# kristi700/ViT-SSL

Measured on AMD Instinct MI355X. Metric: images_per_sec, higher is better.
Workload: dtype bf16; 1 GPU; ViT-B/16 SimMIM 224x224 mask 0.6 dropout 0.1 AdamW, batch 256/GPU; global_batch=256, parallelism=dp1

## Files before the change

vit-ssl_amd/csrc/attention.hip:

```cpp
#include <stdlib.h>
#include "common.h"
#include "attention_tiles.h"
#include "attention_bwd.h"

#ifdef VITSSL_ATTN_STAMPS
__device__ unsigned long long* g_attn_stamps = nullptr;
#define ATTN_STAMP(i)                                                                                   \
  do {                                                                                                  \
    if (g_attn_stamps && threadIdx.x == 0) g_attn_stamps[(size_t)blockIdx.x * 4 + (i)] = __builtin_amdgcn_s_memrealtime(); \
  } while (0)
#else
#define ATTN_STAMP(i) \
  do {                \
  } while (0)
#endif

namespace {

using namespace vitssl_attn;

__device__ __forceinline__ void startup_stagger(int first_round_wgs, int window_ticks) {
  if (window_ticks <= 0 || (int)blockIdx.x >= first_round_wgs) return;
  if (threadIdx.x < 64) {
    const unsigned h = (blockIdx.x * 2654435761u) >> 20;
    const unsigned long long delay = (unsigned long long)window_ticks * h >> 12;
    const unsigned long long t0 = __builtin_amdgcn_s_memrealtime();
    while (__builtin_amdgcn_s_memrealtime() - t0 < delay) __builtin_amdgcn_s_sleep(8);
  }
  __syncthreads();
}


__device__ __forceinline__ f32x4 key_mask_init(int kt, int g, int N) {
  f32x4 v;
#pragma unroll
  for (int r = 0; r < 4; ++r) v[r] = (kt * 16 + 4 * g + r < N) ? 0.f : -INFINITY;
  return v;
}

template <int NKT>
__device__ __forceinline__ void softmax_tile(f32x4 (&s)[NKT], float& m_out, float& sum_out) {
  float m = -INFINITY;
#pragma unroll
  for (int kt = 0; kt < NKT; ++kt) m = fmaxf(fmaxf(m, fmaxf(s[kt][0], s[kt][1])), fmaxf(s[kt][2], s[kt][3]));
  m = fmaxf(m, __shfl_xor(m, 16, 64));
  m = fmaxf(m, __shfl_xor(m, 32, 64));
  const float mc = -m * SCALE_LOG2E;
  const f32x4 c4 = {SCALE_LOG2E, SCALE_LOG2E, SCALE_LOG2E, SCALE_LOG2E}, m4 = {mc, mc, mc, mc};
  f32x4 part = {0.f, 0.f, 0.f, 0.f};
#pragma unroll
  for (int kt = 0; kt < NKT; ++kt) {
    const f32x4 e = __builtin_elementwise_fma(s[kt], c4, m4);
#pragma unroll
    for (int r = 0; r < 4; ++r) s[kt][r] = __builtin_amdgcn_exp2f(e[r]);
    part += s[kt];
  }
  float sum = (part[0] + part[1]) + (part[2] + part[3]);
  sum += __shfl_xor(sum, 16, 64);
  sum += __shfl_xor(sum, 32, 64);
  m_out = m;
  sum_out = sum;
}

template <int NS, int NW>
__global__ __launch_bounds__(64 * NW, 2) void attn_fwd_kernel(const bf16_t* __restrict__ qkv, bf16_t* __restrict__ out,
                                                          float* __restrict__ lse, float* __restrict__ probs, int N, int H,
                                                          int stagger_wgs, int stagger_ticks, unsigned char* __restrict__ out8) {
  extern __shared__ __attribute__((aligned(16))) char smem[];
  constexpr int Np = 32 * NS;
  constexpr int NKT = 2 * NS;
  startup_stagger(stagger_wgs, stagger_ticks);
  char* Kt = smem;
  char* Vt = smem + Np * ROWB;
  const int b = blockIdx.x / H, h = blockIdx.x - b * H;
  const long long stride = 3LL * H * DH;
  const bf16_t* qg = qkv + (long long)b * N * stride + h * DH;
  const bf16_t* kg = qg + (long long)H * DH;
  const bf16_t* vg = kg + (long long)H * DH;
  const int lane = threadIdx.x & 63;
  const int wave = __builtin_amdgcn_readfirstlane(threadIdx.x >> 6);
  const int g = lane >> 4, li = lane & 15;
  const int nqp = (N + 31) >> 5;
  const f32x4 zero4 = {0.f, 0.f, 0.f, 0.f};
  const f32x4 tail0 = key_mask_init(NKT - 2, g, N), tail1 = key_mask_init(NKT - 1, g, N);

  ATTN_STAMP(0);
  bf16x8 qn[2][2];
#pragma unroll
  for (int t = 0; t < 2; ++t) {
    qn[t][0] = glb_frag(qg, stride, wave * 32 + t * 16 + li, 0, N, lane);
    qn[t][1] = glb_frag(qg, stride, wave * 32 + t * 16 + li, 1, N, lane);
  }
  dma_tile<NW>(Kt, kg, stride, N, Np, wave, lane);
  asm volatile("s_waitcnt vmcnt(0)" ::: "memory");
  __builtin_amdgcn_s_barrier();
  dma_tile<NW>(Vt, vg, stride, N, Np, wave, lane);
  ATTN_STAMP(1);

  const int iters = (nqp + NW - 1) / NW;
  for (int it = 0; it < iters; ++it) {
    const int qp = wave + NW * it;
    const bool active = qp < nqp;
    const int q[2] = {qp * 32 + li, qp * 32 + 16 + li};
    bf16x8 qf[2][2];
#pragma unroll
    for (int t = 0; t < 2; ++t) {
      qf[t][0] = qn[t][0];
      qf[t][1] = qn[t][1];
    }
    if (it + 1 < iters) {
#pragma unroll
      for (int t = 0; t < 2; ++t) {
// ... 123 lines not shown
#pragma unroll
    for (int t = 0; t < QT; ++t)
#pragma unroll
      for (int kk = 0; kk < 2; ++kk)
        qq[t][kk] = __builtin_bit_cast(bf16x8, __builtin_amdgcn_raw_buffer_load_b128(
                                                   rq, (unsigned)((long long)q[t] * stride * 2 + 64 * kk + 16 * g), 0, 0));
  };
  constexpr unsigned OOB = 0x80000000u;
  const unsigned out_bytes = (unsigned)((long long)N * H * DH * 2);
  unsigned vrel[4];
  {
    const int tq = (lane >> 2) & 3, tpp = lane & 3;
#pragma unroll
    for (int dt = 0; dt < 4; ++dt) vrel[dt] = (unsigned)(tile_off(4 * g + tq, 2 * dt + (tpp >> 1)) + 8 * (tpp & 1));
  }

  bf16x8 qn[QT][2];
  issue_tiles(item, smem, smem + TILE);
  load_q(item, qn);
  bool first = true;
#ifdef VITSSL_ATTN_STAMPS
  unsigned long long seg[6] = {0, 0, 0, 0, 0, 0};
  unsigned long long tprev = __builtin_amdgcn_s_memrealtime();
#define PSTAMP(i)                                                   \
  do {                                                              \
    __builtin_amdgcn_sched_barrier(0);                              \
    const unsigned long long tn_ = __builtin_amdgcn_s_memrealtime(); \
    seg[i] += tn_ - tprev;                                          \
    tprev = tn_;                                                    \
    __builtin_amdgcn_sched_barrier(0);                              \
  } while (0)
#else
#define PSTAMP(i) \
  do {            \
  } while (0)
#endif

  auto one_item = [&](auto cur_c) {
    constexpr int cur = decltype(cur_c)::value;
    const char* Kt = smem + cur * 2 * TILE;
    const char* Vt = Kt + TILE;
    char* Kn = smem + (cur ^ 1) * 2 * TILE;
    const int b = item / H, h = item - b * H;
    const int next = item + (int)gridDim.x;
    const bool has_next = next < nitems;
    if (probs || first || !active) __builtin_amdgcn_s_waitcnt(0x0F70);
    else if (out8) __builtin_amdgcn_s_waitcnt(0x0F70 | (QT * 7));
    else __builtin_amdgcn_s_waitcnt(0x0F70 | (QT * 3));
    first = false;
    __builtin_amdgcn_s_barrier();
    PSTAMP(0);
    bf16x8 qf[QT][2];
#pragma unroll
    for (int t = 0; t < QT; ++t) {
      qf[t][0] = qn[t][0];
      qf[t][1] = qn[t][1];
    }
    if (has_next) {
      issue_tiles(next, Kn, Kn + TILE);
      load_q(next, qn);
    }
    if (active) {
      f32x4 sc[QT][NKT];
#pragma unroll
      for (int kt = 0; kt < NKT; ++kt) {
        const bf16x8 k0 = lds_frag(Kt, kt * 16 + li, 0, lane);
        const bf16x8 k1 = lds_frag(Kt, kt * 16 + li, 1, lane);
#pragma unroll
        for (int t = 0; t < QT; ++t) sc[t][kt] = MFMA16(k0, qf[t][0], kt == NKT - 2 ? tail0 : (kt == NKT - 1 ? tail1 : zero4));
#pragma unroll
        for (int t = 0; t < QT; ++t) sc[t][kt] = MFMA16(k1, qf[t][1], sc[t][kt]);
      }
      PSTAMP(1);
      float m[QT], sum[QT], inv[QT];
#pragma unroll
      for (int t = 0; t < QT; ++t) softmax_tile<NKT>(sc[t], m[t], sum[t]);
      PSTAMP(2);
      __amdgpu_buffer_rsrc_t rl = __builtin_amdgcn_make_buffer_rsrc((void*)(lse + ((long long)b * H + h) * N), 0, N * 4, 0x00020000);
#pragma unroll
      for (int t = 0; t < QT; ++t) {
        inv[t] = 1.0f / sum[t];
        __builtin_amdgcn_raw_buffer_store_b32(__float_as_uint(m[t] * SCALE + __logf(sum[t])), rl, g == 0 ? (unsigned)q[t] * 4u : OOB, 0, 0);
        if (probs && q[t] < N) {
          int qrow = q[t];
          asm volatile("" : "+v"(qrow));
          float* pr = probs + (((long long)b * H + h) * N + qrow) * N;
#pragma unroll
          for (int kt = 0; kt < NKT; ++kt)
#pragma unroll
            for (int r = 0; r < 4; ++r) {
              const int key = kt * 16 + 4 * g + r;
              if (key < N) pr[key] = sc[t][kt][r] * inv[t];
            }
        }
      }
      f32x4 o[QT][4];
#pragma unroll
      for (int t = 0; t < QT; ++t)
#pragma unroll
        for (int dt = 0; dt < 4; ++dt) o[t][dt] = f32x4{0.f, 0.f, 0.f, 0.f};
      const unsigned vbase = (unsigned)(size_t)LDS_PTR(Vt);
      unsigned va[4];
#pragma unroll
      for (int dt = 0; dt < 4; ++dt) va[dt] = vbase + vrel[dt];
      constexpr int SETS = QT == 2 ? 2 : 1;
      s16x4 lo[SETS][4], hi[SETS][4];
      if constexpr (SETS == 2) tr_read_v4<0>(lo[0], hi[0], va);
      static_for<NS>([&](auto st_c) {
        constexpr int st = decltype(st_c)::value;
        constexpr int set = SETS == 2 ? (st & 1) : 0;
        bf16x8 pf[QT];
#pragma unroll
        for (int t = 0; t < QT; ++t) pf[t] = pack_frag(sc[t][2 * st], sc[t][2 * st + 1]);
        if constexpr (SETS == 1) {
          tr_read_v4<st>(lo[0], hi[0], va);
          asm volatile("s_waitcnt lgkmcnt(0)" ::: "memory");
        } else if constexpr (st + 1 < NS) {
          tr_read_v4<st + 1>(lo[set ^ 1], hi[set ^ 1], va);
          asm volatile("s_waitcnt lgkmcnt(8)" ::: "memory");
        } else {
          asm volatile("s_waitcnt lgkmcnt(0)" ::: "memory");
        }
        __builtin_amdgcn_sched_barrier(0);
#pragma unroll
        for (int dt = 0; dt < 4; ++dt) {
          typedef __attribute__((ext_vector_type(8))) short s16x8;
          const s16x8 v = {lo[set][dt][0], lo[set][dt][1], lo[set][dt][2], lo[set][dt][3], hi[set][dt][0], hi[set][dt][1], hi[set][dt][2], hi[set][dt][3]};
          const bf16x8 vf = __builtin_bit_cast(bf16x8, v);
#pragma unroll
          for (int t = 0; t < QT; ++t) o[t][dt] = MFMA16(vf, pf[t], o[t][dt]);
        }
      });
      PSTAMP(3);
      __amdgpu_buffer_rsrc_t ro = __builtin_amdgcn_make_buffer_rsrc((void*)(out + (long long)b * N * (H * DH)), 0, (int)out_bytes, 0x00020000);
      char* xw = smem + 4 * TILE + wave * 2048;
      const int rho = lane >> 3, kap = lane & 7;
      const unsigned tw = (unsigned)(li * 128 + ((g ^ (2 * (li >> 1))) << 3));
      const unsigned tr = (unsigned)(rho * 128 + ((kap ^ (rho >> 1)) << 4));
#pragma unroll
      for (int t = 0; t < QT; ++t) {
#pragma unroll
        for (int dt = 0; dt < 4; ++dt) *(u32x2*)(xw + (tw ^ (unsigned)(32 * dt))) = pack4(o[t][dt] * inv[t]);
        const u32x4 s1 = *(const u32x4*)(xw + tr), s2 = *(const u32x4*)(xw + ((tr + 1024u) ^ 64u));
        const unsigned rowoff = (unsigned)((wave * QT + t) * 16 + rho) * (unsigned)(H * DH * 2) + (unsigned)(h * DH * 2 + 16 * kap);
        __builtin_amdgcn_raw_buffer_store_b128(s1, ro, rowoff, 0, 0);
        __builtin_amdgcn_raw_buffer_store_b128(s2, ro, rowoff + 8u * (unsigned)(H * DH * 2), 0, 0);
      }
      if (out8) {
        __amdgpu_buffer_rsrc_t r8 = __builtin_amdgcn_make_buffer_rsrc((void*)(out8 + (long long)b * N * (H * DH)), 0, (int)(out_bytes / 2), 0x00020000);
#pragma unroll
        for (int t = 0; t < QT; ++t)
#pragma unroll
          for (int dt = 0; dt < 4; ++dt) {
            const f32x4 v = o[t][dt] * inv[t];
            __builtin_amdgcn_raw_buffer_store_b32(pack_fp8x4(v[0], v[1], v[2], v[3]), r8,
                                                  (unsigned)q[t] * (unsigned)(H * DH) + (unsigned)(h * DH + 4 * g + 16 * dt), 0, 0);
          }
      }
    }
    PSTAMP(4);
#ifdef VITSSL_ATTN_STAMPS
    seg[5] += 1;
#endif
    item = next;
    return has_next;
  };
  for (;;) {
    if (!one_item(IC<0>{})) break;
    if (!one_item(IC<1>{})) break;
  }
#ifdef VITSSL_ATTN_STAMPS
  if (g_attn_stamps && threadIdx.x == 0)
    for (int i = 0; i < 6; ++i) g_attn_stamps[(size_t)blockIdx.x * 8 + i] = seg[i];
#endif
#undef PSTAMP
}

template <int NS, int NW>
__global__ __launch_bounds__(64 * NW, 2) void attn_bwd_fused_kernel(const bf16_t* __restrict__ qkv, const bf16_t* __restrict__ outp,
                                                             const bf16_t* __restrict__ dout, const float* __restrict__ lse,
                                                             bf16_t* __restrict__ dqkv, int N, int H, int stagger_wgs,
                                                             int stagger_ticks, unsigned char* __restrict__ dq8,
                                                             const float* __restrict__ qscale, float* qamax) {
  extern __shared__ __attribute__((aligned(16))) char smem[];
  constexpr int Np = 32 * NS;
  constexpr int SROW = SX_ROW<NS>;
  const float qsc = (dq8 && qscale) ? *qscale : 1.0f;
  float qmax = 0.f;
  startup_stagger(stagger_wgs, stagger_ticks);
  char* Qt = smem;
  char* Dt = Qt + Np * ROWB;
  char* Kt = Dt + Np * ROWB;
  char* Sx = Kt + Np * ROWB;
  float* lse_s = (float*)(Sx + 2 * 32 * SROW);
  float* del_s = lse_s + Np;
  const int b = blockIdx.x / H, h = blockIdx.x - b * H;
  const long long stride = 3LL * H * DH, ostride = (long long)H * DH;
  const bf16_t* qg = qkv + (long long)b * N * stride + h * DH;
  const bf16_t* kg = qg + (long long)H * DH;
  const bf16_t* vg = kg + (long long)H * DH;
  const bf16_t* dog = dout + (long long)b * N * ostride + h * DH;
  const bf16_t* og = outp + (long long)b * N * ostride + h * DH;
  const int lane = threadIdx.x & 63;
  const int wave = __builtin_amdgcn_readfirstlane(threadIdx.x >> 6);
  const int g = lane >> 4, li = lane & 15;
  const bool has_keys = wave < NS;

  ATTN_STAMP(0);
  char* Ot = Sx;
  dma_tile<NW>(Qt, qg, stride, N, Np, wave, lane);
  dma_tile<NW>(Dt, dog, ostride, N, Np, wave, lane);
  dma_tile<NW>(Kt, kg, stride, N, Np, wave, lane);
  dma_tile<NW>(Ot, og, ostride, N, Np, wave, lane);
  bf16x8 kf[2][2], vf[2][2];
  f32x4 kinit[2];
  if (has_keys) {
#pragma unroll
    for (int kt = 0; kt < 2; ++kt) {
      const int key = wave * 32 + kt * 16 + li;
      kinit[kt] = key_mask_init1(key, N);
#pragma unroll
      for (int kk = 0; kk < 2; ++kk) vf[kt][kk] = glb_frag(vg, stride, key, kk, N, lane);
    }
  }
  float lrow[(Np + 32 * NW - 1) / (32 * NW)];
#pragma unroll
  for (int it = 0; it < (Np + 32 * NW - 1) / (32 * NW); ++it) {
    const int row = (threadIdx.x >> 1) + it * 32 * NW;
    lrow[it] = row < N ? lse[((long long)b * H + h) * N + row] : 0.f;
  }
  asm volatile("s_waitcnt vmcnt(0)" ::: "memory");
  __syncthreads();
  if (has_keys) {
#pragma unroll
    for (int kt = 0; kt < 2; ++kt)
#pragma unroll
      for (int kk = 0; kk < 2; ++kk) kf[kt][kk] = lds_frag(Kt, wave * 32 + kt * 16 + li, kk, lane);
  }
#pragma unroll
// ... 349 lines not shown
      }
    }
  }
  dq_tile(Sx + ((NS - 1) & 1) * 32 * SROW, NS - 1);
  ATTN_STAMP(2);
  if (has_keys) {
#pragma unroll
    for (int kt = 0; kt < 2; ++kt) {
      const int key = wave * 32 + kt * 16 + li;
      if (dqkv) {
        char* xw = Qt + wave * 2048;
        const int rho = lane >> 3, kap = lane & 7;
        const unsigned tw = (unsigned)(li * 128 + ((g ^ (2 * (li >> 1))) << 3));
        const unsigned tr = (unsigned)(rho * 128 + ((kap ^ (rho >> 1)) << 4));
        const int key_a = wave * 32 + kt * 16 + rho;
        bf16_t* dka = dqkv + ((long long)b * N + key_a) * stride + (long long)H * DH + h * DH + 8 * kap;
#pragma unroll
        for (int tsel = 0; tsel < 2; ++tsel) {
#pragma unroll
          for (int dt = 0; dt < 4; ++dt) *(u32x2*)(xw + (tw ^ (unsigned)(32 * dt))) = pack4(tsel == 0 ? dk[dt][kt] : dv[dt][kt]);
          const u32x4 s1 = *(const u32x4*)(xw + tr), s2 = *(const u32x4*)(xw + ((tr + 1024u) ^ 64u));
          bf16_t* dst = dka + (long long)tsel * H * DH;
          if (key_a < N) *(u32x4*)dst = s1;
          if (key_a + 8 < N) *(u32x4*)(dst + 8 * stride) = s2;
        }
      }
      if (dq8) {
        unsigned qk[4], qv[4];
#pragma unroll
        for (int dt = 0; dt < 4; ++dt) {
          const f32x4 a = dk[dt][kt], c = dv[dt][kt];
          qk[dt] = pack_fp8x4(a[0] * qsc, a[1] * qsc, a[2] * qsc, a[3] * qsc);
          qv[dt] = pack_fp8x4(c[0] * qsc, c[1] * qsc, c[2] * qsc, c[3] * qsc);
          if (key < N) {
            qmax = fmaxf(qmax, fmaxf(fmaxf(fabsf(a[0]), fabsf(a[1])), fmaxf(fabsf(a[2]), fabsf(a[3]))));
            qmax = fmaxf(qmax, fmaxf(fmaxf(fabsf(c[0]), fabsf(c[1])), fmaxf(fabsf(c[2]), fabsf(c[3]))));
          }
        }
        const u32x4 rk = lane_rows_transpose4(qk), rv = lane_rows_transpose4(qv);
        if (key < N) {
          unsigned char* k8 = dq8 + ((long long)b * N + key) * stride + (long long)H * DH + h * DH + 16 * g;
          *(u32x4*)k8 = rk;
          *(u32x4*)(k8 + (long long)H * DH) = rv;
        }
      }
    }
  }
  if (dq8 && qamax) publish_amax(qmax, qamax, lane);
#ifdef VITSSL_ATTN_STAMPS
  asm volatile("s_waitcnt vmcnt(0)" ::: "memory");
#endif
  ATTN_STAMP(3);
}


template <int NS, bool Q8>
__global__ __launch_bounds__(512) void attn_bwd_pers_kernel(const bf16_t* __restrict__ qkv, const bf16_t* __restrict__ outp,
                                                            const bf16_t* __restrict__ dout, const float* __restrict__ lse,
                                                            bf16_t* __restrict__ dqkv_arg, int N, int H, int nitems,
                                                            unsigned char* __restrict__ dq8_arg, const float* __restrict__ qscale,
                                                            float* qamax) {
  bf16_t* const dqkv = dqkv_arg;
  unsigned char* const dq8 = Q8 ? dq8_arg : nullptr;
  extern __shared__ __attribute__((aligned(16))) char smem[];
  static_assert(NS >= 5 && NS <= 7, "the persistent backward is built for 129-224 tokens");
  constexpr int NW = 8;
  constexpr int Np = 32 * NS;
  constexpr int TILE = Np * ROWB;
  constexpr int SROW = SX_ROW<NS>;
  const float qsc = (Q8 && qscale) ? *qscale : 1.0f;
  float qmax = 0.f;
  char* Qt = smem;
  char* Dt = Qt + TILE;
  char* Kt = Dt + TILE;
  char* Vt = Kt + TILE;
  char* Sx = Vt + TILE;
  float* lse_s = (float*)(Sx + 2 * 32 * SROW);
  float* del_s = lse_s + 2 * Np;
  char* Or = (char*)(del_s + Np);
  const long long stride = 3LL * H * DH, ostride = (long long)H * DH;
  const int lane = threadIdx.x & 63;
  const int wave = __builtin_amdgcn_readfirstlane(threadIdx.x >> 6);
  const int g = lane >> 4, li = lane & 15;
  const bool has_keys = wave < NS;
  const bool delta_wave = wave == NW - 1;
  const int dq_stores = ((!Q8 || dqkv) ? 1 : 0) + (Q8 ? 1 : 0);
  const int G = gridDim.x;
  int item = blockIdx.x;
  if (item >= nitems) return;

  struct Item {
    long long qoff, ooff;
  };
  auto item_of = [&](int it) {
    const int b = it / H, h = it - b * H;
    Item r;
    r.qoff = (long long)b * N * stride + h * DH;
    r.ooff = (long long)b * N * ostride + h * DH;
    return r;
  };
  const int qbytes = (int)((long long)(N - 1) * stride * 2 + ROWB), obytes = (int)((long long)(N - 1) * ostride * 2 + ROWB);
  const int rl8 = lane >> 3;
  const unsigned lane_q = (unsigned)(rl8 * stride * 2 + (((lane & 7) ^ (((rl8 >> 1) & 3) << 1)) << 4));
  const unsigned lane_o = (unsigned)(rl8 * ostride * 2 + (((lane & 7) ^ (((rl8 >> 1) & 3) << 1)) << 4));
  auto dma8 = [&](const bf16_t* base, int total_bytes, long long row_elems, char* lds_rows, unsigned lane_off, int grow0) {
    const long long skip = (long long)grow0 * row_elems * 2;
    const int left = total_bytes > skip ? (int)(total_bytes - skip) : 0;
    __amdgpu_buffer_rsrc_t rs = __builtin_amdgcn_make_buffer_rsrc((void*)(base + (long long)grow0 * row_elems), 0, left, 0x00020000);
    __builtin_amdgcn_raw_ptr_buffer_load_lds(rs, LDS_PTR(lds_rows), 16, lane_off, 0, 0, 0);
  };
  auto issue_slice = [&](const Item& it, int s) {
    const int j = wave & 3;
    const int r0 = 32 * s + 8 * j;
    if (wave < 4) {
      dma8(qkv + it.qoff, qbytes, stride, Qt + r0 * ROWB, lane_q, r0);
      dma8(outp + it.ooff, obytes, ostride, Or + ((s % 3) * 32 + 8 * j) * ROWB, lane_o, r0);
    } else {
      dma8(dout + it.ooff, obytes, ostride, Dt + r0 * ROWB, lane_o, r0);
    }
  };
  auto issue_kv = [&](const Item& it) {
#pragma unroll
    for (int n = 0; n < NS; ++n) {
      const int idx = n * NW + wave;
      const int i = idx >> 1;
      if (idx & 1) dma8(qkv + it.qoff + 2LL * H * DH, qbytes, stride, Vt + i * 8 * ROWB, lane_q, 8 * i);
      else dma8(qkv + it.qoff + (long long)H * DH, qbytes, stride, Kt + i * 8 * ROWB, lane_q, 8 * i);
    }
  };
  auto load_lse = [&](int it, int buf) {
    const int row = threadIdx.x >> 1;
    const float l = row < N ? lse[(long long)it * N + row] : 0.f;
    if ((threadIdx.x & 1) == 0 && row < Np) lse_s[buf * Np + row] = row < N ? l * LOG2E : INFINITY;
  };
  auto delta_slice = [&](int s) { vitssl_attn::delta_slice(del_s, Or, Dt, s, N, lane); };

  Item cur = item_of(item);
  issue_kv(cur);
  issue_slice(cur, 0);
  issue_slice(cur, 1);
  load_lse(item, 0);
  __builtin_amdgcn_s_waitcnt(0x0070);
  __syncthreads();

  const f32x4 c4 = {SCALE_LOG2E, SCALE_LOG2E, SCALE_LOG2E, SCALE_LOG2E}, sc4 = {SCALE, SCALE, SCALE, SCALE};
  const int tq = (lane >> 2) & 3, tpp = lane & 3;
  const unsigned qbase = (unsigned)(size_t)LDS_PTR(Qt);
  unsigned vrel[4];
#pragma unroll
  for (int dt = 0; dt < 4; ++dt) vrel[dt] = qbase + (unsigned)(tile_off(4 * g + tq, 2 * dt + (tpp >> 1)) + 8 * (tpp & 1));
  const int dt_w = wave & 3, qt_w = wave >> 2;
  const unsigned kaddr = vrel[0] - qbase + (unsigned)(size_t)LDS_PTR(Kt) +
                         (unsigned)(tile_off(4 * g + tq, 2 * dt_w + (tpp >> 1)) - tile_off(4 * g + tq, (tpp >> 1)));
  f32x4 kinit[2];
#pragma unroll
  for (int kt = 0; kt < 2; ++kt) kinit[kt] = key_mask_init1(wave * 32 + kt * 16 + li, N);

  for (int par = 0;; par ^= 1) {
    const int next = item + G;
    const bool has_next = next < nitems;
    const float* lse_c = lse_s + par * Np;

    bf16x8 kf[2][2], vf[2][2];
    if (has_keys) {
#pragma unroll
      for (int kt = 0; kt < 2; ++kt)
#pragma unroll
        for (int kk = 0; kk < 2; ++kk) {
          kf[kt][kk] = lds_frag(Kt, wave * 32 + kt * 16 + li, kk, lane);
          vf[kt][kk] = lds_frag(Vt, wave * 32 + kt * 16 + li, kk, lane);
        }
    }
    s16x4 klo[NS], khi[NS];
    load_kt<NS>(klo, khi, kaddr);
    if (delta_wave) delta_slice(0);
    __builtin_amdgcn_s_waitcnt(0xC07F);
    raw_barrier();

    auto dq_tile = [&](const char* sx, int qs) {
      const f32x4 acc = dq_product<NS>(sx, qt_w, g, li, klo, khi);
      const int q = qs * 32 + 16 * qt_w + li;
      const unsigned qoff = (unsigned)q * (unsigned)(stride * 2) + (unsigned)((dt_w * 16 + 4 * g) * 2);
      if (!Q8 || dqkv) {
        __amdgpu_buffer_rsrc_t rsDQ = __builtin_amdgcn_make_buffer_rsrc((void*)(dqkv + cur.qoff), 0, (int)((long long)(N - 1) * stride * 2 + ROWB), 0x00020000);
        __builtin_amdgcn_raw_buffer_store_b64(u32x2{pack_bf2(acc[0], acc[1]), pack_bf2(acc[2], acc[3])}, rsDQ, qoff, 0, 0);
      }
      if constexpr (Q8) {
        __amdgpu_buffer_rsrc_t rsDQ8 = __builtin_amdgcn_make_buffer_rsrc((void*)(dq8 + cur.qoff), 0, (int)((long long)(N - 1) * stride + DH), 0x00020000);
        __builtin_amdgcn_raw_buffer_store_b32(pack_fp8x4(acc[0] * qsc, acc[1] * qsc, acc[2] * qsc, acc[3] * qsc), rsDQ8, qoff >> 1, 0, 0);
        if (q < N) qmax = fmaxf(qmax, fmaxf(fmaxf(fabsf(acc[0]), fabsf(acc[1])), fmaxf(fabsf(acc[2]), fabsf(acc[3]))));
      }
    };

    f32x4 dv[4][2], dk[4][2];
    zero_dkdv(dk, dv);

#pragma unroll 1
    for (int qs = 0; qs < NS; ++qs) {
      char* sx = Sx + (qs & 1) * 32 * SROW;
      int nz = next;
      asm volatile("" : "+s"(nz));
      if (qs + 2 < NS) issue_slice(cur, qs + 2);
      if (qs == NS - 1 && has_next) {
        const Item nx = item_of(nz);
        issue_slice(nx, 0);
        issue_slice(nx, 1);
        load_lse(nz, par ^ 1);
      }
      if (delta_wave && qs + 1 < NS) delta_slice(qs + 1);
      f32x4 p[2][2], ds[2][2];
      if (has_keys) {
        f32x4 a[2][2], c[2][2];
#pragma unroll
        for (int t = 0; t < 2; ++t) {
          const int qrow = qs * 32 + t * 16 + li;
          const bf16x8 qa0 = lds_frag(Qt, qrow, 0, lane), qa1 = lds_frag(Qt, qrow, 1, lane);
          const bf16x8 da0 = lds_frag(Dt, qrow, 0, lane), da1 = lds_frag(Dt, qrow, 1, lane);
#pragma unroll
          for (int kt = 0; kt < 2; ++kt) {
            a[t][kt] = kinit[kt];
            c[t][kt] = f32x4{0.f, 0.f, 0.f, 0.f};
            a[t][kt] = MFMA16(qa0, kf[kt][0], a[t][kt]);
            a[t][kt] = MFMA16(qa1, kf[kt][1], a[t][kt]);
            c[t][kt] = MFMA16(da0, vf[kt][0], c[t][kt]);
            c[t][kt] = MFMA16(da1, vf[kt][1], c[t][kt]);
          }
        }
        if (qs > 0) dq_tile(Sx + ((qs - 1) & 1) * 32 * SROW, qs - 1);
        if (qs == 1 && has_next) issue_kv(item_of(nz));
#pragma unroll
        for (int t = 0; t < 2; ++t) {
          const f32x4 nl = -*(const f32x4*)(lse_c + qs * 32 + t * 16 + 4 * g);
          const f32x4 nd = -*(const f32x4*)(del_s + qs * 32 + t * 16 + 4 * g);
#pragma unroll
          for (int kt = 0; kt < 2; ++kt) {
            const f32x4 e = __builtin_elementwise_fma(a[t][kt], c4, nl);
#pragma unroll
            for (int r = 0; r < 4; ++r) p[t][kt][r] = __builtin_amdgcn_exp2f(e[r]);
            ds[t][kt] = p[t][kt] * __builtin_elementwise_fma(c[t][kt], sc4, nd);
#pragma unroll
            for (int r = 0; r < 4; ++r)
              *(bf16_t*)(sx + (16 * t + 4 * g + r) * SROW + (32 * wave + 16 * kt + li) * 2) = f2bf(ds[t][kt][r]);
          }
        }
      } else {
        if (qs > 0) dq_tile(Sx + ((qs - 1) & 1) * 32 * SROW, qs - 1);
        if (qs == 1 && has_next) issue_kv(item_of(nz));
      }
      const int fly = (qs == 0 ? 0 : dq_stores) + ((qs == 1 && has_next) ? NS : 0);
      switch (fly) {
        case 0: __builtin_amdgcn_s_waitcnt(0x0070); break;
        case 1: __builtin_amdgcn_s_waitcnt(0x0071); break;
        case 2: __builtin_amdgcn_s_waitcnt(0x0072); break;
        case 5: __builtin_amdgcn_s_waitcnt(0x0075); break;
        case 6: __builtin_amdgcn_s_waitcnt(0x0076); break;
        case 7: __builtin_amdgcn_s_waitcnt(0x0077); break;
        case 8: __builtin_amdgcn_s_waitcnt(0x0078); break;
        case 9: __builtin_amdgcn_s_waitcnt(0x0079); break;
        default: __builtin_amdgcn_s_waitcnt(0x0070); break;
      }
      raw_barrier();
      if (has_keys) {
        s16x4 qlo[4], qhi[4], dlo[4], dhi[4];
        const unsigned soff = (unsigned)qs * 4096u;
#pragma unroll
        for (int dt = 0; dt < 4; ++dt) {
          ds_read_tr16<TILE>(dlo[dt], vrel[dt] + soff);
          ds_read_tr16<TILE + 2048>(dhi[dt], vrel[dt] + soff);
        }
#pragma unroll
        for (int dt = 0; dt < 4; ++dt) {
          ds_read_tr16<0>(qlo[dt], vrel[dt] + soff);
          ds_read_tr16<2048>(qhi[dt], vrel[dt] + soff);
        }
        bf16x8 pf[2], sf[2];
#pragma unroll
        for (int kt = 0; kt < 2; ++kt) {
          pf[kt] = pack_frag(p[0][kt], p[1][kt]);
          sf[kt] = pack_frag(ds[0][kt], ds[1][kt]);
        }
        asm volatile("s_waitcnt lgkmcnt(8)" ::: "memory");
        __builtin_amdgcn_sched_barrier(0);
#pragma unroll
        for (int dt = 0; dt < 4; ++dt) {
          const bf16x8 dfr = join_tr(dlo[dt], dhi[dt]);
#pragma unroll
          for (int kt = 0; kt < 2; ++kt) dv[dt][kt] = MFMA16(dfr, pf[kt], dv[dt][kt]);
        }
        asm volatile("s_waitcnt lgkmcnt(0)" ::: "memory");
        __builtin_amdgcn_sched_barrier(0);
#pragma unroll
        for (int dt = 0; dt < 4; ++dt) {
          const bf16x8 qfr = join_tr(qlo[dt], qhi[dt]);
#pragma unroll
          for (int kt = 0; kt < 2; ++kt) dk[dt][kt] = MFMA16(qfr, sf[kt], dk[dt][kt]);
        }
      }
    }
    dq_tile(Sx + ((NS - 1) & 1) * 32 * SROW, NS - 1);
    if (has_keys) {
#pragma unroll
      for (int kt = 0; kt < 2; ++kt) {
        const int key = wave * 32 + kt * 16 + li;
        if (!Q8 || dqkv) {
          char* xw = (wave < 4 ? Qt : Dt) + 64 * ROWB + (wave & 3) * 2048;
          int lz = lane;
          asm volatile("" : "+v"(lz));
          const int rho = lz >> 3, kap = lz & 7, gz = lz >> 4, liz = lz & 15;
          const unsigned tw = (unsigned)(liz * 128 + ((gz ^ (2 * (liz >> 1))) << 3));
          const unsigned tr = (unsigned)(rho * 128 + ((kap ^ (rho >> 1)) << 4));
          const int key_a = wave * 32 + kt * 16 + rho;
          bf16_t* dka = dqkv + cur.qoff + (long long)key_a * stride + (long long)H * DH + 8 * kap;
#pragma unroll
          for (int tsel = 0; tsel < 2; ++tsel) {
#pragma unroll
            for (int dt = 0; dt < 4; ++dt) *(u32x2*)(xw + (tw ^ (unsigned)(32 * dt))) = pack4(tsel == 0 ? dk[dt][kt] : dv[dt][kt]);
            const u32x4 s1 = *(const u32x4*)(xw + tr), s2 = *(const u32x4*)(xw + ((tr + 1024u) ^ 64u));
            bf16_t* dst = dka + (long long)tsel * H * DH;
            if (key_a < N) *(u32x4*)dst = s1;
            if (key_a + 8 < N) *(u32x4*)(dst + 8 * stride) = s2;
          }
        }
        if constexpr (Q8) {
          unsigned qk[4], qv[4];
#pragma unroll
          for (int dt = 0; dt < 4; ++dt) {
            const f32x4 a = dk[dt][kt], c = dv[dt][kt];
            qk[dt] = pack_fp8x4(a[0] * qsc, a[1] * qsc, a[2] * qsc, a[3] * qsc);
            qv[dt] = pack_fp8x4(c[0] * qsc, c[1] * qsc, c[2] * qsc, c[3] * qsc);
            if (key < N) {
              qmax = fmaxf(qmax, fmaxf(fmaxf(fabsf(a[0]), fabsf(a[1])), fmaxf(fabsf(a[2]), fabsf(a[3]))));
              qmax = fmaxf(qmax, fmaxf(fmaxf(fabsf(c[0]), fabsf(c[1])), fmaxf(fabsf(c[2]), fabsf(c[3]))));
            }
          }
          const u32x4 rk = lane_rows_transpose4(qk), rv = lane_rows_transpose4(qv);
          if (key < N) {
            unsigned char* k8 = dq8 + cur.qoff + (long long)key * stride + (long long)H * DH + 16 * g;
            *(u32x4*)k8 = rk;
            *(u32x4*)(k8 + (long long)H * DH) = rv;
          }
        }
      }
    }
    if (!has_next) break;
    item = next;
    cur = item_of(next);
  }
  if (Q8 && qamax) publish_amax(qmax, qamax, lane);
}

int attn_cu_count() { return vitssl_persistent_cus(); }
std::atomic<int> g_last_attn_fwd_grid{0};

int attn_stagger_ticks(int which) {
  static VsEnvInt fwd, bwd;
  return which == 0 ? fwd.get("VITSSL_ATTN_STAGGER_FWD", 0) : bwd.get("VITSSL_ATTN_STAGGER_BWD", 1400);
}

constexpr int ATTN_LDS_LIMIT = 160 * 1024;

template <int NS>
int launch_fwd(const bf16_t* qkv, bf16_t* out, float* lse, float* probs, int B, int N, int H, hipStream_t s,
               unsigned char* out8 = nullptr) {
  if constexpr (NS >= 5) {
    static VsOnce done_p{false};
    const int lds_p = 4 * NS * 32 * ROWB + 8 * 2048;
    const int nitems = B * H;
    const int cus = attn_cu_count();
    const int grid = nitems < cus ? nitems : cus;
    if (int rc = ensure_lds(attn_fwd_pers_kernel<NS, 2>, ATTN_LDS_LIMIT, done_p, "attn_fwd_pers")) return rc;
    g_last_attn_fwd_grid.store(grid, std::memory_order_relaxed);
    hipLaunchKernelGGL((attn_fwd_pers_kernel<NS, 2>), dim3(grid), dim3(512), lds_p, s, qkv, out, lse, probs, N, H, nitems, out8);
    VS_CHECK_LAUNCH("attn_fwd_pers");
  } else {
    constexpr int lds = 2 * NS * 32 * ROWB;
    static_assert(lds <= 48 * 1024, "within the default dynamic-LDS limit");
    constexpr int NW = NS <= 2 ? 2 : 4;
    const int per_cu = lds > 80 * 1024 ? 1 : (lds > 53 * 1024 ? 2 : 3);
    const int cus = attn_cu_count();
    g_last_attn_fwd_grid.store(B * H, std::memory_order_relaxed);
    hipLaunchKernelGGL((attn_fwd_kernel<NS, NW>), dim3(B * H), dim3(64 * NW), lds, s, qkv, out, lse, probs, N, H,
                       cus * per_cu, B * H > 2 * cus * per_cu ? attn_stagger_ticks(0) : 0, out8);
    VS_CHECK_LAUNCH("attn_fwd");
  }
  return VITSSL_OK;
}

template <int NS>
int launch_bwd(const bf16_t* qkv, const bf16_t* out, const bf16_t* dout, const float* lse, bf16_t* dqkv, int B,
               int N, int H, hipStream_t s, unsigned char* dq8 = nullptr, const float* qscale = nullptr, float* qamax = nullptr) {
  const int cus = attn_cu_count();
  if constexpr (NS >= 5 && NS <= 7) {
    static VsOnce done_ps{false}, done_ps8{false};
    constexpr int LDS_PS = 4 * NS * 32 * ROWB + 2 * 32 * (NS * 64 + 16) + 3 * NS * 32 * 4 + 3 * 32 * ROWB;
    static_assert(LDS_PS <= 160 * 1024, "the persistent backward needs four operand tiles in LDS");
    const int nitems = B * H;
    const int grid = nitems < cus ? nitems : cus;
    if (dq8) {
      if (int rc = ensure_lds(attn_bwd_pers_kernel<NS, true>, ATTN_LDS_LIMIT, done_ps8, "attn_bwd_pers")) return rc;
      hipLaunchKernelGGL((attn_bwd_pers_kernel<NS, true>), dim3(grid), dim3(512), LDS_PS, s, qkv, out, dout, lse, dqkv, N, H, nitems, dq8,
                         qscale, qamax);
    } else {
      if (int rc = ensure_lds(attn_bwd_pers_kernel<NS, false>, ATTN_LDS_LIMIT, done_ps, "attn_bwd_pers")) return rc;
      hipLaunchKernelGGL((attn_bwd_pers_kernel<NS, false>), dim3(grid), dim3(512), LDS_PS, s, qkv, out, dout, lse, dqkv, N, H, nitems, dq8,
                         qscale, qamax);
    }
    VS_CHECK_LAUNCH("attn_bwd_pers");
  } else if constexpr (NS == 8) {
    static VsOnce done_p{false};
    const int lds_p = 3 * NS * 32 * ROWB + 2 * 32 * (NS * 64 + 16) + 2 * NS * 32 * 4 + 3 * 32 * ROWB;
    if (int rc = ensure_lds(attn_bwd_pipe_kernel<NS>, ATTN_LDS_LIMIT, done_p, "attn_bwd_pipe")) return rc;
    hipLaunchKernelGGL((attn_bwd_pipe_kernel<NS>), dim3(B * H), dim3(512), lds_p, s, qkv, out, dout, lse, dqkv, N, H,
                       cus, B * H > 2 * cus ? attn_stagger_ticks(1) : 0, dq8, qscale, qamax);
    VS_CHECK_LAUNCH("attn_bwd_pipe");
  } else {
    static_assert(NS <= 4, "the fused backward serves up to 128 tokens");
    constexpr int NW = NS <= 2 ? 2 : 4;
    constexpr int lds_f = 3 * NS * 32 * ROWB + 2 * 32 * (NS * 64 + 16) + 2 * NS * 32 * 4;
    if constexpr (lds_f > 48 * 1024) {
      static VsOnce done_f{false};
      if (int rc = ensure_lds(attn_bwd_fused_kernel<NS, NW>, ATTN_LDS_LIMIT, done_f, "attn_bwd_fused")) return rc;
    }
    const int per_cu = lds_f > 80 * 1024 ? 1 : 2;
    hipLaunchKernelGGL((attn_bwd_fused_kernel<NS, NW>), dim3(B * H), dim3(64 * NW), lds_f, s, qkv, out, dout, lse, dqkv, N, H,
                       cus * per_cu, B * H > 2 * cus * per_cu ? attn_stagger_ticks(1) : 0, dq8, qscale, qamax);
    VS_CHECK_LAUNCH("attn_bwd_fused");
  }
  return VITSSL_OK;
}

#define VS_NS_SWITCH(NSV, CALL)        \
  switch (NSV) {                       \
    case 1: return CALL(1);            \
    case 2: return CALL(2);            \
    case 3: return CALL(3);            \
    case 4: return CALL(4);            \
    case 5: return CALL(5);            \
    case 6: return CALL(6);            \
    case 7: return CALL(7);            \
    default: return CALL(8);           \
  }

int check_attn_shape(const char* who, int B, int N, int H, int dh) {
  VS_CHECK_ARG(B > 0 && N > 0 && H > 0, "%s: empty problem B=%d N=%d H=%d", who, B, N, H);
  VS_CHECK_ARG(dh == DH, "%s: head dim %d unsupported (this build handles dh=64: ViT-Tiny/S/B/L)", who, dh);
  VS_CHECK_ARG(N <= ATTN_LONG_MAX_N, "%s: sequence length %d > %d unsupported", who, N, ATTN_LONG_MAX_N);
  return VITSSL_OK;
}
int check_attn_shape_fp8(const char* who, int B, int N, int H, int dh) {
  if (int rc = check_attn_shape(who, B, N, H, dh)) return rc;
  VS_CHECK_ARG(N <= 256, "%s: sequence length %d > 256 unsupported with fp8 operands (use bf16 operands for up to %d tokens)", who, N,
               ATTN_LONG_MAX_N);
  return VITSSL_OK;
}

}

#ifdef VITSSL_ATTN_STAMPS
extern "C" int vitssl_debug_attn_stamps(void* buf) {
  unsigned long long* p = (unsigned long long*)buf;
  return (int)hipMemcpyToSymbol(HIP_SYMBOL(g_attn_stamps), &p, sizeof(p));
}
#endif

extern "C" int vitssl_debug_last_attn_fwd_grid(void) { return g_last_attn_fwd_grid.load(std::memory_order_relaxed); }

extern "C" int vitssl_attn_fwd(const void* qkv, void* out, float* lse, float* probs, int B, int N, int H, int dh,
                               void* stream) {
  VS_CHECK_ARG(qkv && out && lse, "attn_fwd: null pointer");
  if (int rc = check_attn_shape("attn_fwd", B, N, H, dh)) return rc;
  if (N > 256) {
    int grid = 0;
    const int rc = attn_long_fwd((const bf16_t*)qkv, (bf16_t*)out, lse, probs, B, N, H, (hipStream_t)stream, &grid);
    if (rc == VITSSL_OK) g_last_attn_fwd_grid.store(grid, std::memory_order_relaxed);
    return rc;
// ... 40 lines not shown
```

Measured before the change: 7845 images/s.

## Cut scalar/vector register pressure in attention fwd/bwd via address recomputation

Adds inline-asm helpers that pin values to SGPRs or VGPRs, and uses them to rematerialize lane and wave indices in the forward and persistent backward attention kernels. The backward replaces the per-item struct with incremental (batch, head) counters and uses a 32-bit skip offset per slice for the DMA buffer descriptors. It also restructures issue_kv so each wave loads one K or V column stripe, and simplifies the waitcnt switch. The forward drops the key bound check on non-tail tiles in the probs store and computes the fp8 row from lane layout. An env switch is added to fall back to the non-persistent pipe kernel. The aim is to reduce register pressure and address arithmetic, at the cost of a denser and riskier load schedule.

```diff
diff --git a/vit-ssl_amd/csrc/attention.hip b/vit-ssl_amd/csrc/attention.hip
--- a/vit-ssl_amd/csrc/attention.hip
+++ b/vit-ssl_amd/csrc/attention.hip
@@ -28,6 +28,19 @@
     while (__builtin_amdgcn_s_memrealtime() - t0 < delay) __builtin_amdgcn_s_sleep(8);
   }
   __syncthreads();
+}
+
+__device__ __forceinline__ int here_s(int v) {
+  asm volatile("" : "+s"(v));
+  return v;
+}
+__device__ __forceinline__ unsigned here_s(unsigned v) {
+  asm volatile("" : "+s"(v));
+  return v;
+}
+__device__ __forceinline__ int here_v(int v) {
+  asm volatile("" : "+v"(v));
+  return v;
 }
 
 
@@ -317,15 +330,14 @@
         inv[t] = 1.0f / sum[t];
         __builtin_amdgcn_raw_buffer_store_b32(__float_as_uint(m[t] * SCALE + __logf(sum[t])), rl, g == 0 ? (unsigned)q[t] * 4u : OOB, 0, 0);
         if (probs && q[t] < N) {
-          int qrow = q[t];
-          asm volatile("" : "+v"(qrow));
+          const int qrow = here_v(q[t]), gz = here_v(g);
           float* pr = probs + (((long long)b * H + h) * N + qrow) * N;
 #pragma unroll
           for (int kt = 0; kt < NKT; ++kt)
 #pragma unroll
             for (int r = 0; r < 4; ++r) {
-              const int key = kt * 16 + 4 * g + r;
-              if (key < N) pr[key] = sc[t][kt][r] * inv[t];
+              const int key = kt * 16 + 4 * gz + r;
+              if (kt < NKT - 2 || key < N) pr[key] = sc[t][kt][r] * inv[t];
             }
         }
       }
@@ -369,8 +381,9 @@
       PSTAMP(3);
       __amdgpu_buffer_rsrc_t ro = __builtin_amdgcn_make_buffer_rsrc((void*)(out + (long long)b * N * (H * DH)), 0, (int)out_bytes, 0x00020000);
       char* xw = smem + 4 * TILE + wave * 2048;
-      const int rho = lane >> 3, kap = lane & 7;
-      const unsigned tw = (unsigned)(li * 128 + ((g ^ (2 * (li >> 1))) << 3));
+      const int lz = here_v(lane);
+      const int rho = lz >> 3, kap = lz & 7, gz = lz >> 4, liz = lz & 15;
+      const unsigned tw = (unsigned)(liz * 128 + ((gz ^ (2 * (liz >> 1))) << 3));
       const unsigned tr = (unsigned)(rho * 128 + ((kap ^ (rho >> 1)) << 4));
 #pragma unroll
       for (int t = 0; t < QT; ++t) {
@@ -389,7 +402,7 @@
           for (int dt = 0; dt < 4; ++dt) {
             const f32x4 v = o[t][dt] * inv[t];
             __builtin_amdgcn_raw_buffer_store_b32(pack_fp8x4(v[0], v[1], v[2], v[3]), r8,
-                                                  (unsigned)q[t] * (unsigned)(H * DH) + (unsigned)(h * DH + 4 * g + 16 * dt), 0, 0);
+                                                  (unsigned)((wave * QT + t) * 16 + liz) * (unsigned)(H * DH) + (unsigned)(h * DH + 4 * gz + 16 * dt), 0, 0);
           }
       }
     }
@@ -905,64 +918,65 @@
   const int lane = threadIdx.x & 63;
   const int wave = __builtin_amdgcn_readfirstlane(threadIdx.x >> 6);
   const int g = lane >> 4, li = lane & 15;
-  const bool has_keys = wave < NS;
-  const bool delta_wave = wave == NW - 1;
-  const int dq_stores = ((!Q8 || dqkv) ? 1 : 0) + (Q8 ? 1 : 0);
-  const int G = gridDim.x;
-  int item = blockIdx.x;
-  if (item >= nitems) return;
-
-  struct Item {
-    long long qoff, ooff;
-  };
-  auto item_of = [&](int it) {
-    const int b = it / H, h = it - b * H;
-    Item r;
-    r.qoff = (long long)b * N * stride + h * DH;
-    r.ooff = (long long)b * N * ostride + h * DH;
-    return r;
+  const int dq_stores = Q8 ? (dqkv ? 2 : 1) : 1;
+  if ((int)blockIdx.x >= nitems) return;
+
+  const int gb = (int)gridDim.x / H, gh = (int)gridDim.x - gb * H;
+  const int nbatch = nitems / H;
+  int nb = (int)blockIdx.x / H, nh = (int)blockIdx.x - nb * H;
+  auto item_q = [&](int ib, int ih) { return ((long long)ib * N * 3 * H + ih) * DH; };
+  auto item_o = [&](int ib, int ih) { return ((long long)ib * N * H + ih) * DH; };
+  auto advance = [&] {
+    nb += gb;
+    nh += gh;
+    if (nh >= H) {
+      nh -= H;
+      ++nb;
+    }
   };
   const int qbytes = (int)((long long)(N - 1) * stride * 2 + ROWB), obytes = (int)((long long)(N - 1) * ostride * 2 + ROWB);
+  const unsigned q32 = (unsigned)(64 * stride), o32 = (unsigned)(64 * ostride);
   const int rl8 = lane >> 3;
-  const unsigned lane_q = (unsigned)(rl8 * stride * 2 + (((lane & 7) ^ (((rl8 >> 1) & 3) << 1)) << 4));
-  const unsigned lane_o = (unsigned)(rl8 * ostride * 2 + (((lane & 7) ^ (((rl8 >> 1) & 3) << 1)) << 4));
-  auto dma8 = [&](const bf16_t* base, int total_bytes, long long row_elems, char* lds_rows, unsigned lane_off, int grow0) {
-    const long long skip = (long long)grow0 * row_elems * 2;
-    const int left = total_bytes > skip ? (int)(total_bytes - skip) : 0;
-    __amdgpu_buffer_rsrc_t rs = __builtin_amdgcn_make_buffer_rsrc((void*)(base + (long long)grow0 * row_elems), 0, left, 0x00020000);
+  const unsigned chunk8 = (unsigned)(((lane & 7) ^ (((rl8 >> 1) & 3) << 1)) << 4);
+  const unsigned lane_q = (unsigned)((8 * (wave & 3) + rl8) * stride * 2) + chunk8;
+  const unsigned lane_o = (unsigned)((8 * (wave & 3) + rl8) * ostride * 2) + chunk8;
+  auto dma8 = [&](const bf16_t* base, int total_bytes, unsigned skip, char* lds_rows, unsigned lane_off) {
+    __amdgpu_buffer_rsrc_t rs = __builtin_amdgcn_make_buffer_rsrc((void*)((const char*)base + skip), 0, total_bytes - (int)skip, 0x00020000);
     __builtin_amdgcn_raw_ptr_buffer_load_lds(rs, LDS_PTR(lds_rows), 16, lane_off, 0, 0, 0);
   };
-  auto issue_slice = [&](const Item& it, int s) {
-    const int j = wave & 3;
-    const int r0 = 32 * s + 8 * j;
-    if (wave < 4) {
-      dma8(qkv + it.qoff, qbytes, stride, Qt + r0 * ROWB, lane_q, r0);
-      dma8(outp + it.ooff, obytes, ostride, Or + ((s % 3) * 32 + 8 * j) * ROWB, lane_o, r0);
+  auto issue_slice = [&](long long qoff, long long ooff, int s) {
+    const int wz = here_s(wave);
+    const int j = wz & 3;
+    if (wz < 4) {
+      dma8(qkv + qoff, qbytes, (unsigned)s * q32, Qt + (32 * s + 8 * j) * ROWB, lane_q);
+      dma8(outp + ooff, obytes, (unsigned)s * o32, Or + ((s % 3) * 32 + 8 * j) * ROWB, lane_o);
     } else {
-      dma8(dout + it.ooff, obytes, ostride, Dt + r0 * ROWB, lane_o, r0);
+      dma8(dout + ooff, obytes, (unsigned)s * o32, Dt + (32 * s + 8 * j) * ROWB, lane_o);
     }
   };
-  auto issue_kv = [&](const Item& it) {
-#pragma unroll
-    for (int n = 0; n < NS; ++n) {
-      const int idx = n * NW + wave;
-      const int i = idx >> 1;
-      if (idx & 1) dma8(qkv + it.qoff + 2LL * H * DH, qbytes, stride, Vt + i * 8 * ROWB, lane_q, 8 * i);
-      else dma8(qkv + it.qoff + (long long)H * DH, qbytes, stride, Kt + i * 8 * ROWB, lane_q, 8 * i);
-    }
+  auto issue_kv = [&](long long qoff) {
+    const int wz = here_s(wave);
+    const int j = wz & 3, t = wz >> 2;
+    const unsigned step = here_s(q32);
+    const bf16_t* base = qkv + qoff + (long long)(1 + t) * H * DH;
+    char* dst = Kt + t * TILE + 8 * j * ROWB;
+#pragma unroll
+    for (int n = 0; n < NS; ++n) dma8(base, qbytes, (unsigned)n * step, dst + 32 * n * ROWB, lane_q);
   };
-  auto load_lse = [&](int it, int buf) {
-    const int row = threadIdx.x >> 1;
-    const float l = row < N ? lse[(long long)it * N + row] : 0.f;
-    if ((threadIdx.x & 1) == 0 && row < Np) lse_s[buf * Np + row] = row < N ? l * LOG2E : INFINITY;
+  auto load_lse = [&](int ib, int ih, int buf) {
+    const int tz = here_v((int)threadIdx.x);
+    const int row = tz >> 1;
+    const float l = row < N ? lse[((long long)ib * H + ih) * N + row] : 0.f;
+    if ((tz & 1) == 0 && row < Np) lse_s[buf * Np + row] = row < N ? l * LOG2E : INFINITY;
   };
-  auto delta_slice = [&](int s) { vitssl_attn::delta_slice(del_s, Or, Dt, s, N, lane); };
-
-  Item cur = item_of(item);
-  issue_kv(cur);
-  issue_slice(cur, 0);
-  issue_slice(cur, 1);
-  load_lse(item, 0);
+  auto delta_slice = [&](int s) { vitssl_attn::delta_slice(del_s, Or, Dt, s, N, here_v(lane)); };
+
+  long long cur_q = item_q(nb, nh), cur_o = item_o(nb, nh);
+  issue_kv(cur_q);
+  issue_slice(cur_q, cur_o, 0);
+  issue_slice(cur_q, cur_o, 1);
+  load_lse(nb, nh, 0);
+  advance();
   __builtin_amdgcn_s_waitcnt(0x0070);
   __syncthreads();
 
@@ -980,12 +994,11 @@
   for (int kt = 0; kt < 2; ++kt) kinit[kt] = key_mask_init1(wave * 32 + kt * 16 + li, N);
 
   for (int par = 0;; par ^= 1) {
-    const int next = item + G;
-    const bool has_next = next < nitems;
+    const bool has_next = nb < nbatch;
     const float* lse_c = lse_s + par * Np;
 
     bf16x8 kf[2][2], vf[2][2];
-    if (has_keys) {
+    if (here_s(wave) < NS) {
 #pragma unroll
       for (int kt = 0; kt < 2; ++kt)
 #pragma unroll
@@ -996,7 +1009,7 @@
     }
     s16x4 klo[NS], khi[NS];
     load_kt<NS>(klo, khi, kaddr);
-    if (delta_wave) delta_slice(0);
+    if (here_s(wave) == NW - 1) delta_slice(0);
     __builtin_amdgcn_s_waitcnt(0xC07F);
     raw_barrier();
 
@@ -1005,11 +1018,11 @@
       const int q = qs * 32 + 16 * qt_w + li;
       const unsigned qoff = (unsigned)q * (unsigned)(stride * 2) + (unsigned)((dt_w * 16 + 4 * g) * 2);
       if (!Q8 || dqkv) {
-        __amdgpu_buffer_rsrc_t rsDQ = __builtin_amdgcn_make_buffer_rsrc((void*)(dqkv + cur.qoff), 0, (int)((long long)(N - 1) * stride * 2 + ROWB), 0x00020000);
+        __amdgpu_buffer_rsrc_t rsDQ = __builtin_amdgcn_make_buffer_rsrc((void*)(dqkv + cur_q), 0, qbytes, 0x00020000);
         __builtin_amdgcn_raw_buffer_store_b64(u32x2{pack_bf2(acc[0], acc[1]), pack_bf2(acc[2], acc[3])}, rsDQ, qoff, 0, 0);
       }
       if constexpr (Q8) {
-        __amdgpu_buffer_rsrc_t rsDQ8 = __builtin_amdgcn_make_buffer_rsrc((void*)(dq8 + cur.qoff), 0, (int)((long long)(N - 1) * stride + DH), 0x00020000);
+        __amdgpu_buffer_rsrc_t rsDQ8 = __builtin_amdgcn_make_buffer_rsrc((void*)(dq8 + cur_q), 0, (int)((long long)(N - 1) * stride + DH), 0x00020000);
         __builtin_amdgcn_raw_buffer_store_b32(pack_fp8x4(acc[0] * qsc, acc[1] * qsc, acc[2] * qsc, acc[3] * qsc), rsDQ8, qoff >> 1, 0, 0);
         if (q < N) qmax = fmaxf(qmax, fmaxf(fmaxf(fabsf(acc[0]), fabsf(acc[1])), fmaxf(fabsf(acc[2]), fabsf(acc[3]))));
       }
@@ -1021,14 +1034,15 @@
 #pragma unroll 1
     for (int qs = 0; qs < NS; ++qs) {
       char* sx = Sx + (qs & 1) * 32 * SROW;
-      int nz = next;
-      asm volatile("" : "+s"(nz));
-      if (qs + 2 < NS) issue_slice(cur, qs + 2);
+      const int wq = here_s(wave);
+      const bool has_keys = wq < NS, delta_wave = wq == NW - 1;
+      if (qs + 2 < NS) issue_slice(cur_q, cur_o, qs + 2);
       if (qs == NS - 1 && has_next) {
-        const Item nx = item_of(nz);
-        issue_slice(nx, 0);
-        issue_slice(nx, 1);
-        load_lse(nz, par ^ 1);
+        const int zb = here_s(nb), zh = here_s(nh);
+        const long long nq = item_q(zb, zh), no = item_o(zb, zh);
+        issue_slice(nq, no, 0);
+        issue_slice(nq, no, 1);
+        load_lse(zb, zh, par ^ 1);
       }
       if (delta_wave && qs + 1 < NS) delta_slice(qs + 1);
       f32x4 p[2][2], ds[2][2];
@@ -1050,7 +1064,7 @@
           }
         }
         if (qs > 0) dq_tile(Sx + ((qs - 1) & 1) * 32 * SROW, qs - 1);
-        if (qs == 1 && has_next) issue_kv(item_of(nz));
+        if (qs == 1 && has_next) issue_kv(item_q(here_s(nb), here_s(nh)));
 #pragma unroll
         for (int t = 0; t < 2; ++t) {
           const f32x4 nl = -*(const f32x4*)(lse_c + qs * 32 + t * 16 + 4 * g);
@@ -1068,19 +1082,15 @@
         }
       } else {
         if (qs > 0) dq_tile(Sx + ((qs - 1) & 1) * 32 * SROW, qs - 1);
-        if (qs == 1 && has_next) issue_kv(item_of(nz));
-      }
-      const int fly = (qs == 0 ? 0 : dq_stores) + ((qs == 1 && has_next) ? NS : 0);
-      switch (fly) {
-        case 0: __builtin_amdgcn_s_waitcnt(0x0070); break;
-        case 1: __builtin_amdgcn_s_waitcnt(0x0071); break;
-        case 2: __builtin_amdgcn_s_waitcnt(0x0072); break;
-        case 5: __builtin_amdgcn_s_waitcnt(0x0075); break;
-        case 6: __builtin_amdgcn_s_waitcnt(0x0076); break;
-        case 7: __builtin_amdgcn_s_waitcnt(0x0077); break;
-        case 8: __builtin_amdgcn_s_waitcnt(0x0078); break;
-        case 9: __builtin_amdgcn_s_waitcnt(0x0079); break;
-        default: __builtin_amdgcn_s_waitcnt(0x0070); break;
+        if (qs == 1 && has_next) issue_kv(item_q(here_s(nb), here_s(nh)));
+      }
+      if (qs == 0) __builtin_amdgcn_s_waitcnt(0x0070);
+      else if (qs == 1 && has_next) {
+        if (dq_stores == 1) __builtin_amdgcn_s_waitcnt(0x0070 | (NS + 1));
+        else __builtin_amdgcn_s_waitcnt(0x0070 | (NS + 2));
+      } else {
+        if (dq_stores == 1) __builtin_amdgcn_s_waitcnt(0x0071);
+        else __builtin_amdgcn_s_waitcnt(0x0072);
       }
       raw_barrier();
       if (has_keys) {
@@ -1121,19 +1131,18 @@
       }
     }
     dq_tile(Sx + ((NS - 1) & 1) * 32 * SROW, NS - 1);
-    if (has_keys) {
+    if (here_s(wave) < NS) {
+      const int lz = here_v(lane);
+      const int rho = lz >> 3, kap = lz & 7, gz = lz >> 4, liz = lz & 15;
 #pragma unroll
       for (int kt = 0; kt < 2; ++kt) {
-        const int key = wave * 32 + kt * 16 + li;
+        const int key = wave * 32 + kt * 16 + liz;
         if (!Q8 || dqkv) {
           char* xw = (wave < 4 ? Qt : Dt) + 64 * ROWB + (wave & 3) * 2048;
-          int lz = lane;
-          asm volatile("" : "+v"(lz));
-          const int rho = lz >> 3, kap = lz & 7, gz = lz >> 4, liz = lz & 15;
           const unsigned tw = (unsigned)(liz * 128 + ((gz ^ (2 * (liz >> 1))) << 3));
           const unsigned tr = (unsigned)(rho * 128 + ((kap ^ (rho >> 1)) << 4));
           const int key_a = wave * 32 + kt * 16 + rho;
-          bf16_t* dka = dqkv + cur.qoff + (long long)key_a * stride + (long long)H * DH + 8 * kap;
+          bf16_t* dka = dqkv + cur_q + (long long)key_a * stride + (long long)H * DH + 8 * kap;
 #pragma unroll
           for (int tsel = 0; tsel < 2; ++tsel) {
 #pragma unroll
@@ -1158,7 +1167,7 @@
           }
           const u32x4 rk = lane_rows_transpose4(qk), rv = lane_rows_transpose4(qv);
           if (key < N) {
-            unsigned char* k8 = dq8 + cur.qoff + (long long)key * stride + (long long)H * DH + 16 * g;
+            unsigned char* k8 = dq8 + cur_q + (long long)key * stride + (long long)H * DH + 16 * gz;
             *(u32x4*)k8 = rk;
             *(u32x4*)(k8 + (long long)H * DH) = rv;
           }
@@ -1166,8 +1175,9 @@
       }
     }
     if (!has_next) break;
-    item = next;
-    cur = item_of(next);
+    cur_q = item_q(nb, nh);
+    cur_o = item_o(nb, nh);
+    advance();
   }
   if (Q8 && qamax) publish_amax(qmax, qamax, lane);
 }
@@ -1214,6 +1224,16 @@
                int N, int H, hipStream_t s, unsigned char* dq8 = nullptr, const float* qscale = nullptr, float* qamax = nullptr) {
   const int cus = attn_cu_count();
   if constexpr (NS >= 5 && NS <= 7) {
+    static VsEnvInt persist;
+    if (persist.get("VITSSL_ATTN_BWD_PERSIST", 1) == 0) {
+      static VsOnce done_pp{false};
+      const int lds_p = 3 * NS * 32 * ROWB + 2 * 32 * (NS * 64 + 16) + 2 * NS * 32 * 4 + 3 * 32 * ROWB;
+      if (int rc = ensure_lds(attn_bwd_pipe_kernel<NS>, ATTN_LDS_LIMIT, done_pp, "attn_bwd_pipe")) return rc;
+      hipLaunchKernelGGL((attn_bwd_pipe_kernel<NS>), dim3(B * H), dim3(512), lds_p, s, qkv, out, dout, lse, dqkv, N, H,
+                         cus, B * H > 2 * cus ? attn_stagger_ticks(1) : 0, dq8, qscale, qamax);
+      VS_CHECK_LAUNCH("attn_bwd_pipe");
+      return VITSSL_OK;
+    }
     static VsOnce done_ps{false}, done_ps8{false};
     constexpr int LDS_PS = 4 * NS * 32 * ROWB + 2 * 32 * (NS * 64 + 16) + 3 * NS * 32 * 4 + 3 * 32 * ROWB;
     static_assert(LDS_PS <= 160 * 1024, "the persistent backward needs four operand tiles in LDS");
```

Measured after the change: 7875 images/s, median of 6. No clear change (+0.4%).
